# Shuijing725/CrowdNav_Prediction_AttnGraph

Hardware: AMD Instinct MI355X
Metric: env-steps/sec (sim+policy fwd) at 20 humans (higher is better)
Workload: dtype f32 (big GEMMs as bf16x3 split-precision MFMA, fp32 accumulate); 1 GPU; BASELINE configs[1]: CrowdSimVarNum-v0, 20 humans, 4096 parallel envs per GPU, HH+HR attention on, policy forward + ORCA sim step + auto-reset per step; envs_per_gpu=4096, humans=20, parallelism=dp1 (envs sharded, no rollout collective), policy_init=orthogonal, torch.manual_seed(425), sampled_actions=True, side_stream_tail=inline, dephase_steps=240

## Files before the change

crowdnav_prediction_attngraph_amd/csrc/hh_fused.hip:

```cpp
#include "hh_fused.h"
#include "row_plan.h"

#include <climits>
#include <type_traits>
#include <utility>

namespace {

typedef __bf16 bf16x8 __attribute__((ext_vector_type(8)));
typedef __bf16 bf16x4 __attribute__((ext_vector_type(4)));
typedef float f32x4 __attribute__((ext_vector_type(4)));

__device__ __forceinline__ bf16x8 ldw(const char *p)
{
    return *reinterpret_cast<const bf16x8 *>(p);
}
__device__ __forceinline__ f32x4 mfma(bf16x8 a, bf16x8 b, f32x4 c) { return __builtin_amdgcn_mfma_f32_16x16x32_bf16(a, b, c, 0, 0, 0); }

template <class F, int... I>
__device__ __forceinline__ void static_for_impl(F &&f, std::integer_sequence<int, I...>) { (f(std::integral_constant<int, I>{}), ...); }
template <int N, class F>
__device__ __forceinline__ void static_for(F &&f) { static_for_impl(f, std::make_integer_sequence<int, N>{}); }

struct Split8 { bf16x8 hi, lo; };
__device__ __forceinline__ void split1(float x, __bf16 &hi, __bf16 &lo)
{
    hi = (__bf16)x;
    lo = (__bf16)(x - (float)hi);
}
__device__ __forceinline__ Split8 split8(f32x4 a, f32x4 b)
{
    Split8 s;
#pragma unroll
    for (int q = 0; q < 4; ++q) {
        __bf16 h, l;
        split1(a[q], h, l); s.hi[q] = h; s.lo[q] = l;
        split1(b[q], h, l); s.hi[4 + q] = h; s.lo[4 + q] = l;
    }
    return s;
}

__device__ __forceinline__ int ld_ro(const int *p) { return __hip_atomic_load(p, __ATOMIC_RELAXED, __HIP_MEMORY_SCOPE_WORKGROUP); }

__device__ __forceinline__ int lower_bound_wave(const int *a, int n, int target, int lane)
{
    int lo = 0, hi = n;
    while (hi > lo) {
        const int span = hi - lo, step = (span + 63) >> 6;
        const int idx = lo + lane * step;
        const int v = idx < hi ? ld_ro(a + idx) : INT_MAX;
        const unsigned long long m = __ballot(v >= target);
        const int f = m ? __ffsll(m) - 1 : 64;
        if (f == 0) { hi = lo; }
        else {
            const int nlo = lo + (f - 1) * step + 1;
            int nhi = lo + f * step;
            nhi = nhi < hi ? nhi : hi;
            lo = nlo < nhi ? nlo : nhi; hi = nhi;
        }
    }
    return __builtin_amdgcn_readfirstlane(lo);
}

__device__ __forceinline__ int chunk_boundary(const int *row_off, int E, int total, int c, int n, int lane)
{
    if (c <= 0) return 0;
    if (c >= n) return E;
    const int target = (int)((long long)c * total / n);
    const int e1 = lower_bound_wave(row_off, E, target, lane);
    if (e1 == 0) return 0;
    const int above = ld_ro(row_off + e1) - target, below = target - ld_ro(row_off + e1 - 1);
    return below < above ? e1 - 1 : e1;
}

#ifdef HH_TIMING
__device__ long long *g_hh_tim = nullptr;
#define HH_T(k) do { const long long now_ = clock64(); tacc[k] += now_ - tlast; tlast = now_; } while (0)
#else
#define HH_T(k) do {} while (0)
#endif

struct TileCtx {
    int e_lo, n_env, r0, nrows;
    int my_env, my_start;
    int my_src, my_out;
    int tile_ord;
};

namespace wide {
constexpr int FR = 64;
constexpr int LDS_X = 0;
constexpr int LDS_S = 131072;
constexpr int LDS_H0 = LDS_S, LDS_H1 = LDS_S + 16384;
constexpr int LDS_BYTES = 163840;

template <int NRB>
__device__ __forceinline__ void tile_body(const TileCtx &t, int H, int D, const float *__restrict__ se, const HhFusedWeights &W,
                                          float *__restrict__ out_sp, char *lds, int lane, int wave)
{
    const int i = lane & 15, g = lane >> 4;
    const int loff = lane * 16;
    constexpr int NKS = (NRB + 1) / 2;
#ifdef HH_TIMING
    long long tacc[16] = {0}, tlast = clock64();
#endif

    {
        const int c0 = 32 * wave + 8 * g;
        const float *xp[NRB];
        float v[NRB][8];
#pragma unroll
        for (int rb = 0; rb < NRB; ++rb) {
            int row = rb * 16 + i;
            row = row < t.nrows ? row : t.nrows - 1;
            const int env = __shfl(t.my_env, row, 64), st = __shfl(t.my_start, row, 64);
            xp[rb] = se + ((size_t)(t.e_lo + env) * H + (row - st)) * D;
#pragma unroll
            for (int u = 0; u < 8; ++u) v[rb][u] = W.emb0_b[c0 + u];
        }
        for (int d = 0; d < D; ++d) {
            float w[8];
#pragma unroll
            for (int u = 0; u < 8; ++u) w[u] = W.emb0_w[(c0 + u) * D + d];
#pragma unroll
            for (int rb = 0; rb < NRB; ++rb) {
                const float xd = xp[rb][d];
#pragma unroll
                for (int u = 0; u < 8; ++u) v[rb][u] += xd * w[u];
            }
        }
#pragma unroll
        for (int rb = 0; rb < NRB; ++rb) {
            bf16x8 hi, lo;
#pragma unroll
            for (int u = 0; u < 8; ++u) { __bf16 h, l; split1(fmaxf(v[rb][u], 0.0f), h, l); hi[u] = h; lo[u] = l; }
            *reinterpret_cast<bf16x8 *>(lds + LDS_S + ((0 * 4 + wave) * 4 + rb) * 1024 + loff) = hi;
            *reinterpret_cast<bf16x8 *>(lds + LDS_S + ((1 * 4 + wave) * 4 + rb) * 1024 + loff) = lo;
        }
    }
    HH_T(0);
    __syncthreads();
    HH_T(1);
    {
        const char *wp = (const char *)W.emb2_frag + (size_t)wave * 4 * 16 * 1024 + loff;
#pragma unroll 1
        for (int half = 0; half < 2; ++half) {
            f32x4 acc[4][NRB];
#pragma unroll
            for (int j = 0; j < 4; ++j)
#pragma unroll
                for (int rb = 0; rb < NRB; ++rb) acc[j][rb] = f32x4{0.f, 0.f, 0.f, 0.f};
            bf16x8 wq[2][8];
#pragma unroll
            for (int j = 0; j < 4; ++j) {
                wq[0][2 * j] = ldw(wp + ((0 * 8 + half * 4 + j) * 2 + 0) * 1024);
                wq[0][2 * j + 1] = ldw(wp + ((0 * 8 + half * 4 + j) * 2 + 1) * 1024);
            }
#pragma unroll
            for (int ks = 0; ks < 4; ++ks) {
                if (ks + 1 < 4) {
#pragma unroll
                    for (int j = 0; j < 4; ++j) {
                        wq[(ks + 1) & 1][2 * j] = ldw(wp + (((ks + 1) * 8 + half * 4 + j) * 2 + 0) * 1024);
                        wq[(ks + 1) & 1][2 * j + 1] = ldw(wp + (((ks + 1) * 8 + half * 4 + j) * 2 + 1) * 1024);
                    }
                }
                bf16x8 xh[NRB], xl[NRB];
#pragma unroll
// ... 281 lines not shown
    }
    __syncthreads();
    HH_T(15);
#ifdef HH_TIMING
    if (g_hh_tim && wave == 0 && lane == 0) {
        long long *d = g_hh_tim + (size_t)blockIdx.x * 20;
        for (int k = 0; k < 16; ++k) d[k] += tacc[k];
        d[16] += 1; d[17] += t.nrows; d[18] += NRB;
        long long *d2 = g_hh_tim + (size_t)256 * 20 + ((size_t)blockIdx.x * 4 + (t.tile_ord < 3 ? t.tile_ord : 3)) * 4;
        d2[0] += tacc[4]; d2[1] += NRB; d2[2] += 1;
    }
#endif
}
}

template <int NT>
__device__ __forceinline__ void row_offsets_prologue(int E, int H, const float *__restrict__ det, int *row_off, unsigned long long *live_total, char *lds)
{
    constexpr int NW = NT / 64;
    int *part = reinterpret_cast<int *>(lds);
    const int tid = threadIdx.x, ln = tid & 63, wv = tid >> 6;
    const int chunk = (E + NT - 1) / NT;
    const int lo = tid * chunk < E ? tid * chunk : E, hi = lo + chunk < E ? lo + chunk : E;
    int sum = 0;
    for (int e = lo; e < hi; ++e) { int nd = (int)det[e]; nd = nd < 1 ? 1 : (nd > H ? H : nd); sum += nd; }
    int incl = sum;
#pragma unroll
    for (int o = 1; o < 64; o <<= 1) {
        const int v = __shfl_up(incl, o, 64);
        if (ln >= o) incl += v;
    }
    if (ln == 63) part[wv] = incl;
    __syncthreads();
    int run = incl - sum;
    for (int w = 0; w < wv; ++w) run += part[w];
    for (int e = lo; e < hi; ++e) {
        row_off[e] = run;
        int nd = (int)det[e]; nd = nd < 1 ? 1 : (nd > H ? H : nd);
        run += nd;
    }
    if (tid == NT - 1) {
        row_off[E] = run;
        if (live_total && blockIdx.x == 0) *live_total += (unsigned long long)run;
    }
    (void)NW;
    __builtin_amdgcn_fence(__ATOMIC_RELEASE, "workgroup");
    __syncthreads();
    __builtin_amdgcn_fence(__ATOMIC_ACQUIRE, "workgroup");
}

template <int FR>
__device__ __forceinline__ TileCtx next_tile(const int *row_off, int e, int e_end, int chunk_end_row, int tile_ord, int lane)
{
    TileCtx t;
    t.tile_ord = tile_ord;
    t.e_lo = e;
    t.r0 = ld_ro(row_off + e);
    const int probe = e + 1 + lane;
    const int v = probe <= e_end ? ld_ro(row_off + probe) : INT_MAX;
    const int left = chunk_end_row - t.r0;
    const int ntile = (left + FR - 1) / FR;
    const int rows = v == INT_MAX ? INT_MAX : v - t.r0;
    const bool ok = rows <= FR && left - rows <= FR * (ntile - 1);
    const int rest = left - rows;
    int key = ok ? ((((rows + 15) >> 4) + ((rest + 15) >> 4)) << 8) + (FR - rows) : INT_MAX;
    int best = key;
#pragma unroll
    for (int o = 32; o > 0; o >>= 1) { const int x = __shfl_xor(best, o, 64); best = x < best ? x : best; }
    int n_env;
    if (best == INT_MAX) {
        n_env = __popcll(__ballot(rows <= FR));
        n_env = n_env < 1 ? 1 : n_env;
    } else {
        n_env = __ffsll(__ballot(key == best));
    }
    t.n_env = n_env;
    t.nrows = __builtin_amdgcn_readfirstlane(__shfl(v, n_env - 1, 64)) - t.r0;
    const int prev_end = __shfl(v, lane >= 1 ? lane - 1 : 0, 64);
    const int st = lane >= n_env ? INT_MAX : (lane == 0 ? 0 : prev_end - t.r0);
    int cnt = 0;
    for (int k = 0; k < n_env; ++k) cnt += lane >= __builtin_amdgcn_readlane(st, k) ? 1 : 0;
    t.my_env = lane < t.nrows ? cnt - 1 : -1;
    t.my_start = __shfl(st, cnt - 1 >= 0 ? cnt - 1 : 0, 64);
    t.my_src = 0; t.my_out = t.r0 + lane;
    return t;
}

struct PlanPre { int it, out0; };
__device__ __forceinline__ PlanPre plan_prefetch(const int32_t *plan, int E, int tile, int lane)
{
    PlanPre p;
    p.it = (plan + rp_off_items(E))[(size_t)tile * 64 + lane];
    p.out0 = (plan + rp_off_rowoff())[p.it & 0xffff];
    return p;
}
__device__ __forceinline__ TileCtx plan_tile(const PlanPre &pre, int H, int tile_ord, int lane)
{
    TileCtx t;
    const unsigned long long zero = __ballot((pre.it >> 16) == 0);
    const int cnt = zero ? __ffsll((long long)zero) - 1 : 64;
    const int it = lane < cnt ? pre.it : 0;
    const int rows = it >> 16, id = it & 0xffff;
    const int out0 = pre.out0;
    int incl = rows;
#pragma unroll
    for (int o = 1; o < 64; o <<= 1) { const int y = __shfl_up(incl, o, 64); if (lane >= o) incl += y; }
    const int st = lane < cnt ? incl - rows : INT_MAX;
    t.tile_ord = tile_ord; t.e_lo = 0; t.r0 = 0; t.n_env = cnt;
    t.nrows = __builtin_amdgcn_readfirstlane(__shfl(incl, 63, 64));
    int c = 0;
    for (int k = 0; k < cnt; ++k) c += lane >= __builtin_amdgcn_readlane(st, k) ? 1 : 0;
    const int me = c - 1 >= 0 ? c - 1 : 0;
    t.my_env = lane < t.nrows ? c - 1 : -1;
    t.my_start = __shfl(st, me, 64);
    const int off = lane - t.my_start;
    t.my_src = __shfl(id, me, 64) * H + off;
    t.my_out = __shfl(out0, me, 64) + off;
    return t;
}

__global__ __launch_bounds__(256, 1) void hh_fused_wide_kernel(int E, int H, int D, const float *__restrict__ se, const float *__restrict__ det,
                                                               int *row_off, unsigned long long *live_total, HhFusedWeights W, float *__restrict__ out_sp,
                                                               unsigned long long *stamp)
{
    const CnStampScope stamp_scope(stamp);
    extern __shared__ __attribute__((aligned(16))) char lds[];
    if (det) row_offsets_prologue<256>(E, H, det, row_off, live_total, lds);
    if (stamp && blockIdx.x == 0 && threadIdx.x == 0) stamp[1] = (unsigned long long)row_off[E];
    if (W.prio) __builtin_amdgcn_s_setprio(3);
    const int lane = threadIdx.x & 63, wave = __builtin_amdgcn_readfirstlane(threadIdx.x >> 6);
    const int total = ld_ro(row_off + E);
    int e = chunk_boundary(row_off, E, total, (int)blockIdx.x, (int)gridDim.x, lane);
    const int e_end = chunk_boundary(row_off, E, total, (int)blockIdx.x + 1, (int)gridDim.x, lane);
    if (e >= e_end) return;
    int tile_ord = 0;
    const int chunk_end_row = ld_ro(row_off + e_end);
    while (e < e_end) {
        const TileCtx t = next_tile<wide::FR>(row_off, e, e_end, chunk_end_row, tile_ord++, lane);
        const int nrb = (t.nrows + 15) >> 4;
        switch (nrb) {
        case 1: wide::tile_body<1>(t, H, D, se, W, out_sp, lds, lane, wave); break;
        case 2: wide::tile_body<2>(t, H, D, se, W, out_sp, lds, lane, wave); break;
        case 3: wide::tile_body<3>(t, H, D, se, W, out_sp, lds, lane, wave); break;
        default: wide::tile_body<4>(t, H, D, se, W, out_sp, lds, lane, wave); break;
        }
        e += t.n_env;
    }
}

namespace team {

constexpr int FR = 63;
constexpr int LDS_BYTES = 163840;
template <int RB_>
struct Layout {
    static constexpr int RB = RB_;
    static constexpr bool TURNS = RB_ == 4;
    static constexpr int X_PLANE = 16 * RB * 1024;
    static constexpr int LDS_X = 0;
    static constexpr int LDS_S = 2 * X_PLANE;
    static constexpr int H_PLANE = 2 * RB * 1024;
    static constexpr int H_BYTES = 2 * H_PLANE;
    static constexpr int TEAM_S = TURNS ? 0 : 2 * H_BYTES;
    static constexpr int E0_PLANE = 4 * RB * 1024;
    static constexpr int XCH_TEAM = 4 * 2 * RB * 1024;
    static constexpr int CTR = TURNS ? LDS_X + X_PLANE + (15 * RB + 3) * 1024 + 63 * 16 : LDS_S + 4 * H_BYTES;
    static_assert(LDS_S + (TURNS ? 2 : 4) * H_BYTES + (TURNS ? 0 : 16) <= LDS_BYTES, "layout exceeds the LDS");
};

typedef __attribute__((address_space(3))) unsigned lds_u32;

typedef int i32x4 __attribute__((ext_vector_type(4)));
struct WeightBuf {
    __amdgpu_buffer_rsrc_t rs;
    unsigned emb2, qkv, os;
};
__device__ __forceinline__ WeightBuf make_weight_buf(const HhFusedWeights &W)
{
    const char *a = (const char *)W.emb2_frag, *b = (const char *)W.qkv_frag, *c = (const char *)W.os_frag;
    const char *lo = a < b ? a : b; lo = lo < c ? lo : c;
    WeightBuf wb;
    wb.rs = __builtin_amdgcn_make_buffer_rsrc((void *)lo, 0, 0x7fffffff, 0x00020000);
    wb.emb2 = (unsigned)(a - lo); wb.qkv = (unsigned)(b - lo); wb.os = (unsigned)(c - lo);
    return wb;
}
__device__ __forceinline__ bf16x8 ldb(const WeightBuf &wb, unsigned soff, unsigned voff)
{
    return __builtin_bit_cast(bf16x8, __builtin_amdgcn_raw_buffer_load_b128(wb.rs, voff, soff, 0));
}

struct RowBuf { __amdgpu_buffer_rsrc_t rs; };
__device__ __forceinline__ RowBuf make_row_buf(float *base, int r0, int nrows, int width)
{
    RowBuf rb;
    rb.rs = __builtin_amdgcn_make_buffer_rsrc((void *)(base + (size_t)r0 * width), 0, nrows * width * 4, 0x00020000);
    return rb;
}
constexpr int TRAIN_STORE_AUX = 2;
__device__ __forceinline__ void st4(const RowBuf &b, int float_off, f32x4 v)
{
    __builtin_amdgcn_raw_buffer_store_b128(__builtin_bit_cast(i32x4, v), b.rs, float_off * 4, 0, TRAIN_STORE_AUX);
}
__device__ __forceinline__ void st1(const RowBuf &b, int float_off, float v)
{
    __builtin_amdgcn_raw_buffer_store_b32(__builtin_bit_cast(int, v), b.rs, float_off * 4, 0, TRAIN_STORE_AUX);
}

__device__ __forceinline__ void team_barrier(char *lds, int bar_off, unsigned &target, int lane)
{
    lds_u32 *ctr = (lds_u32 *)(lds + bar_off);
    target += 4;
    asm volatile("s_waitcnt lgkmcnt(0)" ::: "memory");
    if (lane == 0) __hip_atomic_fetch_add(ctr, 1u, __ATOMIC_RELAXED, __HIP_MEMORY_SCOPE_WORKGROUP);
    while ((int)(__builtin_amdgcn_readfirstlane(__hip_atomic_load(ctr, __ATOMIC_RELAXED, __HIP_MEMORY_SCOPE_WORKGROUP)) - target) < 0)
        __builtin_amdgcn_s_sleep(1);
    asm volatile("" ::: "memory");
}

__device__ __forceinline__ void wait_turn(char *lds, int ctr_off, unsigned turn)
{
    lds_u32 *done = (lds_u32 *)(lds + ctr_off + 8);
    const unsigned need = 4u * turn;
    while ((int)(__builtin_amdgcn_readfirstlane(__hip_atomic_load(done, __ATOMIC_RELAXED, __HIP_MEMORY_SCOPE_WORKGROUP)) - need) < 0)
        __builtin_amdgcn_s_sleep(1);
    asm volatile("" ::: "memory");
}
__device__ __forceinline__ void finish_turn(char *lds, int ctr_off, int lane)
{
    lds_u32 *done = (lds_u32 *)(lds + ctr_off + 8);
    asm volatile("s_waitcnt lgkmcnt(0)" ::: "memory");
    if (lane == 0) __hip_atomic_fetch_add(done, 1u, __ATOMIC_RELAXED, __HIP_MEMORY_SCOPE_WORKGROUP);
}

template <int NRB, int J0, int RB>
__device__ __forceinline__ void finish_rows(const TileCtx &t, const f32x4 (&acc)[4][NRB], const char *xch, const HhFusedWeights &W,
                                            float *__restrict__ out_sp, int lane, int wave, const f32x4 *bpre = nullptr)
{
    const int i = lane & 15, g = lane >> 4, loff = lane * 16;
#pragma unroll
    for (int jj = 0; jj < 2; ++jj) {
        const int f0 = (4 * wave + J0 + jj) * 16 + 4 * g;
        const f32x4 b = bpre ? bpre[jj] : *reinterpret_cast<const f32x4 *>(W.os_b + f0);
#pragma unroll
        for (int rb = 0; rb < NRB; ++rb) {
            const f32x4 other = *reinterpret_cast<const f32x4 *>(xch + ((wave * 2 + jj) * RB + rb) * 1024 + loff);
            const int row = rb * 16 + i;
            const int orow = __shfl(t.my_out, row, 64);
            if (row < t.nrows) {
                f32x4 v = acc[J0 + jj][rb] + other + b;
#pragma unroll
                for (int q = 0; q < 4; ++q) v[q] = fmaxf(v[q], 0.0f);
                __builtin_nontemporal_store(v, reinterpret_cast<f32x4 *>(out_sp + (size_t)orow * 256 + f0));
            }
        }
    }
}

constexpr int PF = 2;

template <int NRB, bool TRAIN>
__device__ __forceinline__ void tile_body(const TileCtx &t, int H, int D, const float *__restrict__ se, const HhFusedWeights &W, const WeightBuf &WB,
                                          float *__restrict__ out_sp, char *lds, int lane_in, int wave, int tm)
{
    using L = Layout<(NRB <= 3 ? 3 : 4)>;
    constexpr int RB = L::RB, X_PLANE = L::X_PLANE, LDS_X = L::LDS_X, LDS_S = L::LDS_S, H_PLANE = L::H_PLANE, H_BYTES = L::H_BYTES,
                  E0_PLANE = L::E0_PLANE, XCH_TEAM = L::XCH_TEAM, LDS_CTR = L::CTR;
    int lane = lane_in;
    asm volatile("" : "+v"(lane));
    const int i = lane & 15, g = lane >> 4;
    const int loff = lane * 16;
    const unsigned uoff = (unsigned)loff;
    RowBuf o_e0{}, o_x{}, o_qkv{}, o_attn{};
    if (TRAIN) {
        o_e0 = make_row_buf(W.e0_out, t.r0, t.nrows, 128); o_x = make_row_buf(W.x_out, t.r0, t.nrows, 512);
        o_qkv = make_row_buf(W.qkv_out, t.r0, t.nrows, 1536); o_attn = make_row_buf(W.attn_out, t.r0, t.nrows, 512);
    }
    constexpr int NKS = (NRB + 1) / 2;
    const int w8 = 4 * tm + wave;
    RowBuf BB;
    BB.rs = __builtin_amdgcn_make_buffer_rsrc((void *)W.qkv_b, 0, 1536 * 4, 0x00020000);
#ifdef HH_TIMING
    long long tacc[16] = {0}, tlast = clock64();
#endif

    if (w8 == 0 && lane < 4) *reinterpret_cast<unsigned *>(lds + LDS_CTR + 4 * lane) = 0u;
    unsigned bar_target = 0;
    bf16x8 wq[4][8];
    {
        const int wv = w8 >> 1, half = w8 & 1;
        const unsigned wp = WB.emb2 + (unsigned)wv * 4 * 16 * 1024;
#pragma unroll
        for (int ks = 0; ks < 4; ++ks)
#pragma unroll
            for (int j = 0; j < 4; ++j) {
                wq[ks][2 * j] = ldb(WB, wp + ((ks * 8 + half * 4 + j) * 2 + 0) * 1024, uoff);
                wq[ks][2 * j + 1] = ldb(WB, wp + ((ks * 8 + half * 4 + j) * 2 + 1) * 1024, uoff);
            }
    }
    {
        const int c0 = 32 * wave + 8 * g;
#pragma unroll
        for (int rr = 0; rr < (NRB + 1) / 2; ++rr) {
            const int rb = 2 * rr + tm;
            if (rb < NRB) {
                int row = rb * 16 + i;
                row = row < t.nrows ? row : t.nrows - 1;
                const float *xp = se + (size_t)__shfl(t.my_src, row, 64) * D;
                float v[8];
#pragma unroll
                for (int u = 0; u < 8; ++u) v[u] = W.emb0_b[c0 + u];
                for (int d = 0; d < D; ++d) {
                    const float xd = xp[d];
#pragma unroll
                    for (int u = 0; u < 8; ++u) v[u] += xd * W.emb0_w[(c0 + u) * D + d];
                }
                bf16x8 hi, lo;
#pragma unroll
                for (int u = 0; u < 8; ++u) { v[u] = fmaxf(v[u], 0.0f); __bf16 h, l; split1(v[u], h, l); hi[u] = h; lo[u] = l; }
                if (TRAIN) {
                    st4(o_e0, (rb * 16 + i) * 128 + c0, f32x4{v[0], v[1], v[2], v[3]});
                    st4(o_e0, (rb * 16 + i) * 128 + c0 + 4, f32x4{v[4], v[5], v[6], v[7]});
                }
                *reinterpret_cast<bf16x8 *>(lds + LDS_S + (wave * RB + rb) * 1024 + loff) = hi;
                *reinterpret_cast<bf16x8 *>(lds + LDS_S + E0_PLANE + (wave * RB + rb) * 1024 + loff) = lo;
            }
        }
    }
    __syncthreads();
    HH_T(0);
    {
        f32x4 acc[4][NRB];
#pragma unroll
        for (int j = 0; j < 4; ++j)
#pragma unroll
            for (int rb = 0; rb < NRB; ++rb) acc[j][rb] = f32x4{0.f, 0.f, 0.f, 0.f};
#pragma unroll
        for (int ks = 0; ks < 4; ++ks) {
            bf16x8 xh[NRB], xl[NRB];
#pragma unroll
            for (int rb = 0; rb < NRB; ++rb) {
                xh[rb] = *reinterpret_cast<const bf16x8 *>(lds + LDS_S + (ks * RB + rb) * 1024 + loff);
                xl[rb] = *reinterpret_cast<const bf16x8 *>(lds + LDS_S + E0_PLANE + (ks * RB + rb) * 1024 + loff);
            }
            __builtin_amdgcn_sched_barrier(0);
            const bf16x8 *w = wq[ks];
#pragma unroll
            for (int j = 0; j < 4; ++j)
#pragma unroll
                for (int rb = 0; rb < NRB; ++rb) acc[j][rb] = mfma(w[2 * j + 1], xh[rb], acc[j][rb]);
#pragma unroll
            for (int j = 0; j < 4; ++j)
#pragma unroll
                for (int rb = 0; rb < NRB; ++rb) acc[j][rb] = mfma(w[2 * j], xl[rb], acc[j][rb]);
#pragma unroll
            for (int j = 0; j < 4; ++j)
#pragma unroll
                for (int rb = 0; rb < NRB; ++rb) acc[j][rb] = mfma(w[2 * j], xh[rb], acc[j][rb]);
            __builtin_amdgcn_sched_barrier(0);
        }
#pragma unroll
        for (int p = 0; p < 2; ++p) {
            const int fb0 = 4 * w8 + 2 * p;
            const f32x4 ba = *reinterpret_cast<const f32x4 *>(W.emb2_b + fb0 * 16 + 4 * g);
            const f32x4 bb = *reinterpret_cast<const f32x4 *>(W.emb2_b + (fb0 + 1) * 16 + 4 * g);
            const int kx = 2 * w8 + p;
#pragma unroll
            for (int rb = 0; rb < NRB; ++rb) {
                f32x4 a = acc[2 * p][rb] + ba, b = acc[2 * p + 1][rb] + bb;
#pragma unroll
                for (int q = 0; q < 4; ++q) { a[q] = fmaxf(a[q], 0.0f); b[q] = fmaxf(b[q], 0.0f); }
                if (TRAIN) {
                    st4(o_x, (rb * 16 + i) * 512 + fb0 * 16 + 4 * g, a);
                    st4(o_x, (rb * 16 + i) * 512 + fb0 * 16 + 4 * g + 16, b);
                }
                const Split8 s = split8(a, b);
                *reinterpret_cast<bf16x8 *>(lds + LDS_X + (kx * RB + rb) * 1024 + loff) = s.hi;
                if (!(L::TURNS && rb == 3 && kx == 15 && lane == 63))
                    *reinterpret_cast<bf16x8 *>(lds + LDS_X + X_PLANE + (kx * RB + rb) * 1024 + loff) = s.lo;
            }
        }
    }
    __syncthreads();
    HH_T(1);

    unsigned vmask = 0;
    {
        const int q = 16 * wave + i;
        const int eq = __shfl(t.my_env, q, 64);
#pragma unroll
        for (int jb = 0; jb < NRB; ++jb)
#pragma unroll
            for (int r = 0; r < 4; ++r) {
                const int ek = __shfl(t.my_env, 16 * jb + 4 * g + r, 64);
                if (ek == eq && eq >= 0) vmask |= 1u << (jb * 4 + r);
            }
    }

    f32x4 acc_os[4][NRB];
#pragma unroll
    for (int j = 0; j < 4; ++j)
#pragma unroll
        for (int rb = 0; rb < NRB; ++rb) acc_os[j][rb] = f32x4{0.f, 0.f, 0.f, 0.f};

    char *const H0 = lds + LDS_S + tm * L::TEAM_S, *const H1 = H0 + H_BYTES;
    const int bar = LDS_CTR + 4 * tm;
    const int h0 = ((int)blockIdx.x >> 3) & 7;
    bf16x8 wf[PF][6];
    auto ring_prologue = [&](const int hh_) __attribute__((always_inline)) {
        const unsigned wp_ = WB.qkv + (unsigned)((((h0 + 2 * hh_ + tm) & 7) * 4 + wave) * 16) * 6 * 1024;
#pragma unroll
        for (int p = 0; p < PF - 1; ++p)
#pragma unroll
            for (int c = 0; c < 6; ++c) wf[p][c] = ldb(WB, wp_ + (p * 6 + c) * 1024, uoff);
    };
    ring_prologue(0);
#pragma unroll 1
    for (int hh = 0; hh < 4; ++hh) {
        const int h = (h0 + 2 * hh + tm) & 7;
        f32x4 aq[NRB], ak[NRB], av[NRB];
#pragma unroll
        for (int rb = 0; rb < NRB; ++rb) { aq[rb] = f32x4{0.f, 0.f, 0.f, 0.f}; ak[rb] = aq[rb]; av[rb] = aq[rb]; }
        const unsigned wp = WB.qkv + (unsigned)((h * 4 + wave) * 16) * 6 * 1024;
        f32x4 bq_pf, bk_pf; float bv_pf;
        bf16x8 xh[2][NRB], xl[2][NRB];
#pragma unroll
        for (int rb = 0; rb < NRB; ++rb) {
            xh[0][rb] = *reinterpret_cast<const bf16x8 *>(lds + LDS_X + rb * 1024 + loff);
            xl[0][rb] = *reinterpret_cast<const bf16x8 *>(lds + LDS_X + X_PLANE + rb * 1024 + loff);
        }
        static_assert(16 % PF == 0, "the ring position must be compile-time inside the unrolled group");
        auto group = [&](const int k4, auto tail_c) __attribute__((always_inline)) {
        constexpr bool TAIL = decltype(tail_c)::value;
        static_for<PF>([&](auto ku_c) __attribute__((always_inline)) {
            constexpr int ku = decltype(ku_c)::value;
            const int ks = k4 + ku;
            {
                if (!TAIL || ku == 0) {
#pragma unroll
                    for (int c = 0; c < 6; ++c) wf[(ku + PF - 1) % PF][c] = ldb(WB, wp + ((ks + PF - 1) * 6 + c) * 1024, uoff);
                }
                if (!TAIL || ku + 1 < PF) {
#pragma unroll
// ... 150 lines not shown
        if (wave < NRB) {
#pragma unroll
            for (int ks = 0; ks < NKS; ++ks) {
                const Split8 sp = split8(f32x4{p[2 * ks][0], p[2 * ks][1], p[2 * ks][2], p[2 * ks][3]},
                                         f32x4{p[2 * ks + 1][0], p[2 * ks + 1][1], p[2 * ks + 1][2], p[2 * ks + 1][3]});
                *reinterpret_cast<bf16x8 *>(H0 + (ks * RB + wave) * 1024 + loff) = sp.hi;
                *reinterpret_cast<bf16x8 *>(H0 + H_PLANE + (ks * RB + wave) * 1024 + loff) = sp.lo;
            }
        }
        team_barrier(lds, bar, bar_target, lane);
        HH_T(7);
        f32x4 o[NRB];
#pragma unroll
        for (int ib = 0; ib < NRB; ++ib) o[ib] = f32x4{0.f, 0.f, 0.f, 0.f};
#pragma unroll
        for (int ks = 0; ks < NKS; ++ks) {
            const Split8 vf = split8(av[2 * ks], 2 * ks + 1 < NRB ? av[2 * ks + 1 < NRB ? 2 * ks + 1 : 0] : f32x4{0.f, 0.f, 0.f, 0.f});
#pragma unroll
            for (int ib = 0; ib < NRB; ++ib) {
                const bf16x8 ph = *reinterpret_cast<const bf16x8 *>(H0 + (ks * RB + ib) * 1024 + loff);
                const bf16x8 pl = *reinterpret_cast<const bf16x8 *>(H0 + H_PLANE + (ks * RB + ib) * 1024 + loff);
                o[ib] = mfma(vf.lo, ph, o[ib]);
                o[ib] = mfma(vf.hi, pl, o[ib]);
                o[ib] = mfma(vf.hi, ph, o[ib]);
            }
        }
#pragma unroll
        for (int ib = 0; ib < NRB; ++ib) {
            if (TRAIN) st4(o_attn, (ib * 16 + i) * 512 + h * 64 + 16 * wave + 4 * g, o[ib]);
            bf16x4 oh, ol;
#pragma unroll
            for (int q = 0; q < 4; ++q) { __bf16 a, b; split1(o[ib][q], a, b); oh[q] = a; ol[q] = b; }
            const int off = ((wave >> 1) * RB + ib) * 1024 + loff + 8 * (wave & 1);
            *reinterpret_cast<bf16x4 *>(H1 + off) = oh;
            *reinterpret_cast<bf16x4 *>(H1 + H_PLANE + off) = ol;
        }
        HH_T(8);
        team_barrier(lds, bar, bar_target, lane);
        HH_T(9);
#pragma unroll
        for (int ks = 0; ks < 2; ++ks) {
            bf16x8 oh[NRB], ol[NRB];
#pragma unroll
            for (int rb = 0; rb < NRB; ++rb) {
                oh[rb] = *reinterpret_cast<const bf16x8 *>(H1 + (ks * RB + rb) * 1024 + loff);
                ol[rb] = *reinterpret_cast<const bf16x8 *>(H1 + H_PLANE + (ks * RB + rb) * 1024 + loff);
            }
#pragma unroll
            for (int j = 0; j < 4; ++j)
#pragma unroll
                for (int rb = 0; rb < NRB; ++rb) acc_os[j][rb] = mfma(wos[ks][j][1], oh[rb], acc_os[j][rb]);
#pragma unroll
            for (int j = 0; j < 4; ++j)
#pragma unroll
                for (int rb = 0; rb < NRB; ++rb) acc_os[j][rb] = mfma(wos[ks][j][0], ol[rb], acc_os[j][rb]);
#pragma unroll
            for (int j = 0; j < 4; ++j)
#pragma unroll
                for (int rb = 0; rb < NRB; ++rb) acc_os[j][rb] = mfma(wos[ks][j][0], oh[rb], acc_os[j][rb]);
            if (L::TURNS && ks == 1) finish_turn(lds, LDS_CTR, lane);
        }
        __builtin_amdgcn_s_setprio(1);
        HH_T(10);
    }
    f32x4 bfin[2];
#pragma unroll
    for (int jj = 0; jj < 2; ++jj) bfin[jj] = *reinterpret_cast<const f32x4 *>(W.os_b + (4 * wave + 2 * tm + jj) * 16 + 4 * g);
    __syncthreads();
    HH_T(11);
    {
        char *const xch = lds + LDS_X;
        if (tm == 0) {
#pragma unroll
            for (int jj = 0; jj < 2; ++jj)
#pragma unroll
                for (int rb = 0; rb < NRB; ++rb) *reinterpret_cast<f32x4 *>(xch + ((wave * 2 + jj) * RB + rb) * 1024 + loff) = acc_os[2 + jj][rb];
        } else {
#pragma unroll
            for (int jj = 0; jj < 2; ++jj)
#pragma unroll
                for (int rb = 0; rb < NRB; ++rb) *reinterpret_cast<f32x4 *>(xch + XCH_TEAM + ((wave * 2 + jj) * RB + rb) * 1024 + loff) = acc_os[jj][rb];
        }
        __syncthreads();
        if (tm == 0) finish_rows<NRB, 0, RB>(t, acc_os, xch + XCH_TEAM, W, out_sp, lane, wave, bfin);
        else finish_rows<NRB, 2, RB>(t, acc_os, xch, W, out_sp, lane, wave, bfin);
    }
    HH_T(12);
#ifdef HH_TIMING
    if (g_hh_tim && wave == 0 && lane == 0) {
        long long *d = g_hh_tim + ((size_t)blockIdx.x * 2 + tm) * 20;
        for (int k = 0; k < 16; ++k) d[k] += tacc[k];
        d[16] += 1; d[17] += t.nrows; d[18] += NRB;
    }
#endif
}

}

template <bool TRAIN>
__global__ __launch_bounds__(512, 2) void hh_fused_kernel(int E, int H, int D, const float *__restrict__ se, const float *__restrict__ det,
                                                          int *row_off, unsigned long long *live_total, HhFusedWeights W, float *__restrict__ out_sp,
                                                          const int32_t *__restrict__ plan, unsigned long long *stamp)
{
    const CnStampScope stamp_scope(TRAIN ? nullptr : stamp);
    extern __shared__ __attribute__((aligned(16))) char lds[];
#ifdef HH_TIMING
    const long long k_c0 = clock64(), k_r0 = wall_clock64();
#endif
    bool planned = !TRAIN && det && rp_usable(plan, E, H) && plan[1] == (int)gridDim.x;
    if (planned) {
        const int32_t *pro = plan + rp_off_rowoff();
        int bad = 0;
        for (int i = (int)threadIdx.x; i < E; i += (int)blockDim.x) {
            int nd = (int)det[i]; nd = nd < 1 ? 1 : (nd > H ? H : nd);
            bad |= (pro[i + 1] - pro[i]) ^ nd;
        }
        volatile int *flag = reinterpret_cast<volatile int *>(lds);
        if (threadIdx.x == 0) *flag = 0;
        __syncthreads();
        if (__ballot(bad != 0) != 0ull && (threadIdx.x & 63) == 0) *flag = 1;
        __syncthreads();
        planned = __builtin_amdgcn_readfirstlane(*flag) == 0;
        __syncthreads();
    }
    if (det && !planned) row_offsets_prologue<512>(E, H, det, row_off, live_total, lds);
    if (!TRAIN && stamp && blockIdx.x == 0 && threadIdx.x == 0) stamp[1] = (unsigned long long)(planned ? plan[3] : row_off[E]);
#ifdef HH_TIMING
    const long long k_c1 = clock64();
#endif
    __builtin_amdgcn_s_setprio(1);
    const int lane = threadIdx.x & 63, w8 = __builtin_amdgcn_readfirstlane(threadIdx.x >> 6);
    const int wave = w8 & 3, tm = w8 >> 2;
    int e = 0, e_end = 0, chunk_end_row = 0, n_plan = 0;
    PlanPre pre{0, 0};
    if (planned) {
        if (live_total && blockIdx.x == 0 && threadIdx.x == 0) *live_total += (unsigned long long)plan[3];
        n_plan = plan[2];
        pre = plan_prefetch(plan, E, (int)blockIdx.x, lane);
        for (int i = (int)(blockIdx.x * blockDim.x + threadIdx.x); i <= E; i += (int)(gridDim.x * blockDim.x)) row_off[i] = plan[rp_off_rowoff() + i];
    } else {
        const int total = ld_ro(row_off + E);
        e = chunk_boundary(row_off, E, total, (int)blockIdx.x, (int)gridDim.x, lane);
        e_end = chunk_boundary(row_off, E, total, (int)blockIdx.x + 1, (int)gridDim.x, lane);
        if (e >= e_end) return;
        chunk_end_row = ld_ro(row_off + e_end);
    }
    int tile_ord = 0;
    const team::WeightBuf WB = team::make_weight_buf(W);
    for (;;) {
        TileCtx t;
        if (planned) {
            if (tile_ord >= n_plan) break;
            const PlanPre cur = pre;
            ++tile_ord;
            if (tile_ord < n_plan) pre = plan_prefetch(plan, E, (int)blockIdx.x + tile_ord * (int)gridDim.x, lane);
            t = plan_tile(cur, H, tile_ord - 1, lane);
            if (t.nrows == 0) continue;
        } else {
            if (e >= e_end) break;
            t = next_tile<team::FR>(row_off, e, e_end, chunk_end_row, tile_ord++, lane);
            t.my_src = (t.e_lo + t.my_env) * H + (lane - t.my_start);
            e += t.n_env;
        }
        const int nrb = (t.nrows + 15) >> 4;
        switch (nrb) {
        case 1: team::tile_body<1, TRAIN>(t, H, D, se, W, WB, out_sp, lds, lane, wave, tm); break;
        case 2: team::tile_body<2, TRAIN>(t, H, D, se, W, WB, out_sp, lds, lane, wave, tm); break;
        case 3: team::tile_body<3, TRAIN>(t, H, D, se, W, WB, out_sp, lds, lane, wave, tm); break;
        default: team::tile_body<4, TRAIN>(t, H, D, se, W, WB, out_sp, lds, lane, wave, tm); break;
        }
    }
#ifdef HH_TIMING
    if (g_hh_tim && (threadIdx.x & 255) == 0) {
        long long *d = g_hh_tim + ((size_t)blockIdx.x * 2 + (threadIdx.x >> 8)) * 20;
        d[13] += clock64() - k_c0; d[14] += wall_clock64() - k_r0; d[15] += k_c1 - k_c0;
    }
#endif
}

__device__ __forceinline__ int koff(int g, int u, bool perm) { return perm ? 16 * (u >> 2) + 4 * g + (u & 3) : 8 * g + u; }

__device__ __forceinline__ void bake_emb2(int idx, const float *__restrict__ w, __bf16 *__restrict__ out)
{
    if (idx >= 512 * 128) return;
    const int u = idx & 7, lane = (idx >> 3) & 63, j = (idx >> 9) & 7, ks = (idx >> 12) & 3, wv = idx >> 14;
    const int fb = 8 * wv + j;
    const float x = w[(size_t)(fb * 16 + (lane & 15)) * 128 + 32 * ks + koff(lane >> 4, u, false)];
    const __bf16 hi = (__bf16)x;
    const size_t base = ((((size_t)wv * 4 + ks) * 8 + j) * 2) * 512 + lane * 8 + u;
    out[base] = hi;
    out[base + 512] = (__bf16)(x - (float)hi);
}
__device__ __forceinline__ void bake_qkv(int idx, const float *__restrict__ w, __bf16 *__restrict__ out)
{
    if (idx >= 1536 * 512) return;
    const int u = idx & 7, lane = (idx >> 3) & 63;
    int rest = idx >> 9;
    const int j = rest % 3; rest /= 3;
    const int ks = rest & 15, wv = (rest >> 4) & 3, h = rest >> 6;
    const int sec = j == 2 ? 2 : (wv & 1), blk = j == 2 ? wv : (wv & ~1) + j;
    const float x = w[(size_t)(sec * 512 + h * 64 + 16 * blk + (lane & 15)) * 512 + 32 * ks + koff(lane >> 4, u, true)];
    const __bf16 hi = (__bf16)x;
    const size_t base = (((((size_t)h * 4 + wv) * 16 + ks) * 3 + j) * 2) * 512 + lane * 8 + u;
    out[base] = hi;
    out[base + 512] = (__bf16)(x - (float)hi);
}
__device__ __forceinline__ void bake_os(int idx, const float *__restrict__ w, __bf16 *__restrict__ out)
{
    if (idx >= 256 * 512) return;
    const int u = idx & 7, lane = (idx >> 3) & 63, j = (idx >> 9) & 3, ks = (idx >> 11) & 1, wv = (idx >> 12) & 3, h = idx >> 14;
    const float x = w[(size_t)((4 * wv + j) * 16 + (lane & 15)) * 512 + h * 64 + 32 * ks + koff(lane >> 4, u, true)];
    const __bf16 hi = (__bf16)x;
    const size_t base = (((((size_t)h * 4 + wv) * 2 + ks) * 4 + j) * 2) * 512 + lane * 8 + u;
    out[base] = hi;
    out[base + 512] = (__bf16)(x - (float)hi);
}

__global__ void bake_all_kernel(const float *__restrict__ emb2_w, const float *__restrict__ qkv_w, const float *__restrict__ os_w, __bf16 *__restrict__ emb2_frag,
                                __bf16 *__restrict__ qkv_frag, __bf16 *__restrict__ os_frag)
{
    constexpr int B1 = 512 * 128 / 256, B2 = B1 + 1536 * 512 / 256;
    const int b = blockIdx.x;
    if (b < B1) bake_emb2(b * 256 + (int)threadIdx.x, emb2_w, emb2_frag);
    else if (b < B2) bake_qkv((b - B1) * 256 + (int)threadIdx.x, qkv_w, qkv_frag);
    else bake_os((b - B2) * 256 + (int)threadIdx.x, os_w, os_frag);
}

}

int hh_fused_bake(const float *emb2_w, const float *qkv_w, const float *os_w, void *emb2_frag, void *qkv_frag, void *os_frag, hipStream_t st)
{
    hipLaunchKernelGGL(bake_all_kernel, dim3((512 * 128 + 1536 * 512 + 256 * 512) / 256), dim3(256), 0, st, emb2_w, qkv_w, os_w, (__bf16 *)emb2_frag, (__bf16 *)qkv_frag,
                       (__bf16 *)os_frag);
    CN_CHECK_LAUNCH();
    return CN_OK;
}

#ifdef HH_TIMING
extern "C" int cn_hh_fused_set_timing(long long *buf)
{
    CN_HIP(hipMemcpyToSymbol(HIP_SYMBOL(g_hh_tim), &buf, sizeof(buf)));
    return CN_OK;
}
#endif

int hh_fused_forward(int E, int H, int D, const float *spatial_edges, const float *det, int *row_off, unsigned long long *live_total,
                     const HhFusedWeights &w, float *out_sp, hipStream_t st, const int32_t *row_plan)
{
    unsigned long long *stamp = cn_stamp_slot(CN_K_HH_FUSED);
    static thread_local int attr_dev = -1;
    int dev = 0;
    CN_HIP(hipGetDevice(&dev));
    if (dev != attr_dev) {
// ... 20 lines not shown
```

Baseline: 15.56 million env-steps/s.

## Overlap plan and emb0 loads with weight fetch in team HH kernel

Moves the next tile's plan-item load and the output-row-offset lookup into the tile body, issuing them early so their latency hides behind the emb2 weight loads and first MFMAs. The per-row emb0 input/weight loads are hoisted and batched across row blocks with software pipelining before the weight-register loads. The kernel prologue's plan validation now loads det and row offsets into registers in a fixed unrolled batch and uses a per-wave flag array instead of a strided loop with three barriers. The cost is higher register pressure and more complex scheduling with sched_barrier and held() pins.

```diff
diff --git a/crowdnav_prediction_attngraph_amd/csrc/hh_fused.hip b/crowdnav_prediction_attngraph_amd/csrc/hh_fused.hip
--- a/crowdnav_prediction_attngraph_amd/csrc/hh_fused.hip
+++ b/crowdnav_prediction_attngraph_amd/csrc/hh_fused.hip
@@ -83,7 +83,8 @@
 struct TileCtx {
     int e_lo, n_env, r0, nrows;
     int my_env, my_start;
-    int my_src, my_out;
+    int my_src;
+    int out0, it;
     int tile_ord;
 };
 
@@ -531,26 +532,19 @@
     for (int k = 0; k < n_env; ++k) cnt += lane >= __builtin_amdgcn_readlane(st, k) ? 1 : 0;
     t.my_env = lane < t.nrows ? cnt - 1 : -1;
     t.my_start = __shfl(st, cnt - 1 >= 0 ? cnt - 1 : 0, 64);
-    t.my_src = 0; t.my_out = t.r0 + lane;
+    t.my_src = 0;
+    t.out0 = t.r0 + (lane < n_env ? st : 0); t.it = 0;
     return t;
 }
 
-struct PlanPre { int it, out0; };
-__device__ __forceinline__ PlanPre plan_prefetch(const int32_t *plan, int E, int tile, int lane)
-{
-    PlanPre p;
-    p.it = (plan + rp_off_items(E))[(size_t)tile * 64 + lane];
-    p.out0 = (plan + rp_off_rowoff())[p.it & 0xffff];
-    return p;
-}
-__device__ __forceinline__ TileCtx plan_tile(const PlanPre &pre, int H, int tile_ord, int lane)
+constexpr int PLAN_NONE = -2, PLAN_LAST = -1;
+__device__ __forceinline__ TileCtx plan_tile(int item, int H, int tile_ord, int lane)
 {
     TileCtx t;
-    const unsigned long long zero = __ballot((pre.it >> 16) == 0);
+    const unsigned long long zero = __ballot((item >> 16) == 0);
     const int cnt = zero ? __ffsll((long long)zero) - 1 : 64;
-    const int it = lane < cnt ? pre.it : 0;
+    const int it = lane < cnt ? item : 0;
     const int rows = it >> 16, id = it & 0xffff;
-    const int out0 = pre.out0;
     int incl = rows;
 #pragma unroll
     for (int o = 1; o < 64; o <<= 1) { const int y = __shfl_up(incl, o, 64); if (lane >= o) incl += y; }
@@ -564,7 +558,7 @@
     t.my_start = __shfl(st, me, 64);
     const int off = lane - t.my_start;
     t.my_src = __shfl(id, me, 64) * H + off;
-    t.my_out = __shfl(out0, me, 64) + off;
+    t.out0 = 0; t.it = item;
     return t;
 }
 
@@ -682,7 +676,7 @@
 }
 
 template <int NRB, int J0, int RB>
-__device__ __forceinline__ void finish_rows(const TileCtx &t, const f32x4 (&acc)[4][NRB], const char *xch, const HhFusedWeights &W,
+__device__ __forceinline__ void finish_rows(const TileCtx &t, int my_out, const f32x4 (&acc)[4][NRB], const char *xch, const HhFusedWeights &W,
                                             float *__restrict__ out_sp, int lane, int wave, const f32x4 *bpre = nullptr)
 {
     const int i = lane & 15, g = lane >> 4, loff = lane * 16;
@@ -694,7 +688,7 @@
         for (int rb = 0; rb < NRB; ++rb) {
             const f32x4 other = *reinterpret_cast<const f32x4 *>(xch + ((wave * 2 + jj) * RB + rb) * 1024 + loff);
             const int row = rb * 16 + i;
-            const int orow = __shfl(t.my_out, row, 64);
+            const int orow = __shfl(my_out, row, 64);
             if (row < t.nrows) {
                 f32x4 v = acc[J0 + jj][rb] + other + b;
 #pragma unroll
@@ -709,7 +703,7 @@
 
 template <int NRB, bool TRAIN>
 __device__ __forceinline__ void tile_body(const TileCtx &t, int H, int D, const float *__restrict__ se, const HhFusedWeights &W, const WeightBuf &WB,
-                                          float *__restrict__ out_sp, char *lds, int lane_in, int wave, int tm)
+                                          float *__restrict__ out_sp, char *lds, int lane_in, int wave, int tm, const int32_t *__restrict__ plan, int plan_next, int &it_next)
 {
     using L = Layout<(NRB <= 3 ? 3 : 4)>;
     constexpr int RB = L::RB, X_PLANE = L::X_PLANE, LDS_X = L::LDS_X, LDS_S = L::LDS_S, H_PLANE = L::H_PLANE, H_BYTES = L::H_BYTES,
@@ -734,10 +728,56 @@
 
     if (w8 == 0 && lane < 4) *reinterpret_cast<unsigned *>(lds + LDS_CTR + 4 * lane) = 0u;
     unsigned bar_target = 0;
+    constexpr int NRR = (NRB + 1) / 2;
+    const int c0 = 32 * wave + 8 * g;
+    const float *xp[NRR];
+    float v[NRR][8];
+    float xv[NRR][4], wv[8][4], bv0[8];
+    auto e0_load = [&](const int d0, const int q0, const int q1) __attribute__((always_inline)) {
+#pragma unroll
+        for (int q = q0; q < q1; ++q) {
+#pragma unroll
+            for (int rr = 0; rr < NRR; ++rr) xv[rr][q] = xp[rr][d0 + q];
+#pragma unroll
+            for (int u = 0; u < 8; ++u) wv[u][q] = W.emb0_w[(c0 + u) * D + d0 + q];
+        }
+    };
+    auto e0_fma = [&](const int q0, const int q1) __attribute__((always_inline)) {
+#pragma unroll
+        for (int q = q0; q < q1; ++q)
+#pragma unroll
+            for (int rr = 0; rr < NRR; ++rr)
+#pragma unroll
+                for (int u = 0; u < 8; ++u) v[rr][u] += xv[rr][q] * wv[u][q];
+    };
+#pragma unroll
+    for (int rr = 0; rr < NRR; ++rr) {
+        int row = (2 * rr + tm) * 16 + i;
+        row = row < t.nrows ? row : t.nrows - 1;
+        xp[rr] = se + (size_t)__shfl(t.my_src, row, 64) * D;
+    }
+#pragma unroll
+    for (int q = 0; q < 4; ++q) {
+#pragma unroll
+        for (int rr = 0; rr < NRR; ++rr) xv[rr][q] = 0.0f;
+#pragma unroll
+        for (int u = 0; u < 8; ++u) wv[u][q] = 0.0f;
+    }
+    {
+        const int q1 = D >= 2 ? 1 : 0;
+#pragma unroll
+        for (int rr = 0; rr < NRR; ++rr) { xv[rr][0] = xp[rr][0]; xv[rr][1] = xp[rr][q1]; }
+#pragma unroll
+        for (int u = 0; u < 8; ++u) { wv[u][0] = W.emb0_w[(c0 + u) * D]; wv[u][1] = W.emb0_w[(c0 + u) * D + q1]; }
+    }
+    if (D >= 4) e0_load(0, 2, 4);
+#pragma unroll
+    for (int u = 0; u < 8; ++u) bv0[u] = W.emb0_b[c0 + u];
+    __builtin_amdgcn_sched_barrier(0);
     bf16x8 wq[4][8];
     {
-        const int wv = w8 >> 1, half = w8 & 1;
-        const unsigned wp = WB.emb2 + (unsigned)wv * 4 * 16 * 1024;
+        const int wv_ = w8 >> 1, half = w8 & 1;
+        const unsigned wp = WB.emb2 + (unsigned)wv_ * 4 * 16 * 1024;
 #pragma unroll
         for (int ks = 0; ks < 4; ++ks)
 #pragma unroll
@@ -746,29 +786,47 @@
                 wq[ks][2 * j + 1] = ldb(WB, wp + ((ks * 8 + half * 4 + j) * 2 + 1) * 1024, uoff);
             }
     }
+    int out0_ld, it_ld;
+    const int pnext = TRAIN ? PLAN_NONE : __builtin_amdgcn_readfirstlane(plan_next);
+    const bool has_plan = pnext != PLAN_NONE, has_next = pnext >= 0;
     {
-        const int c0 = 32 * wave + 8 * g;
-#pragma unroll
-        for (int rr = 0; rr < (NRB + 1) / 2; ++rr) {
+        const int32_t *dummy = reinterpret_cast<const int32_t *>(se);
+        out0_ld = *(has_plan ? plan + rp_off_rowoff() + (t.it & 0xffff) : dummy);
+        it_ld = *(has_next ? plan + pnext + lane : dummy);
+    }
+    __builtin_amdgcn_sched_barrier(0);
+#pragma unroll
+    for (int rr = 0; rr < NRR; ++rr)
+#pragma unroll
+        for (int q = 0; q < 4; ++q) xv[rr][q] = held(xv[rr][q]);
+#pragma unroll
+    for (int u = 0; u < 8; ++u) {
+        bv0[u] = held(bv0[u]);
+#pragma unroll
+        for (int q = 0; q < 4; ++q) wv[u][q] = held(wv[u][q]);
+    }
+    {
+#pragma unroll
+        for (int rr = 0; rr < NRR; ++rr)
+#pragma unroll
+            for (int u = 0; u < 8; ++u) v[rr][u] = bv0[u];
+        e0_fma(0, 1);
+        if (D >= 2) e0_fma(1, 2);
+        if (D >= 4) e0_fma(2, 4);
+        int d0 = 4;
+        for (; d0 + 4 <= D; d0 += 4) { e0_load(d0, 0, 4); e0_fma(0, 4); }
+        if (d0 + 2 <= D) { e0_load(d0, 0, 2); e0_fma(0, 2); }
+        if ((D & 1) && D > 1) { e0_load(D - 1, 0, 1); e0_fma(0, 1); }
+#pragma unroll
+        for (int rr = 0; rr < NRR; ++rr) {
             const int rb = 2 * rr + tm;
             if (rb < NRB) {
-                int row = rb * 16 + i;
-                row = row < t.nrows ? row : t.nrows - 1;
-                const float *xp = se + (size_t)__shfl(t.my_src, row, 64) * D;
-                float v[8];
-#pragma unroll
-                for (int u = 0; u < 8; ++u) v[u] = W.emb0_b[c0 + u];
-                for (int d = 0; d < D; ++d) {
-                    const float xd = xp[d];
-#pragma unroll
-                    for (int u = 0; u < 8; ++u) v[u] += xd * W.emb0_w[(c0 + u) * D + d];
-                }
                 bf16x8 hi, lo;
 #pragma unroll
-                for (int u = 0; u < 8; ++u) { v[u] = fmaxf(v[u], 0.0f); __bf16 h, l; split1(v[u], h, l); hi[u] = h; lo[u] = l; }
+                for (int u = 0; u < 8; ++u) { v[rr][u] = fmaxf(v[rr][u], 0.0f); __bf16 h, l; split1(v[rr][u], h, l); hi[u] = h; lo[u] = l; }
                 if (TRAIN) {
-                    st4(o_e0, (rb * 16 + i) * 128 + c0, f32x4{v[0], v[1], v[2], v[3]});
-                    st4(o_e0, (rb * 16 + i) * 128 + c0 + 4, f32x4{v[4], v[5], v[6], v[7]});
+                    st4(o_e0, (rb * 16 + i) * 128 + c0, f32x4{v[rr][0], v[rr][1], v[rr][2], v[rr][3]});
+                    st4(o_e0, (rb * 16 + i) * 128 + c0 + 4, f32x4{v[rr][4], v[rr][5], v[rr][6], v[rr][7]});
                 }
                 *reinterpret_cast<bf16x8 *>(lds + LDS_S + (wave * RB + rb) * 1024 + loff) = hi;
                 *reinterpret_cast<bf16x8 *>(lds + LDS_S + E0_PLANE + (wave * RB + rb) * 1024 + loff) = lo;
@@ -777,6 +835,7 @@
     }
     __syncthreads();
     HH_T(0);
+    int my_out;
     {
         f32x4 acc[4][NRB];
 #pragma unroll
@@ -807,6 +866,9 @@
                 for (int rb = 0; rb < NRB; ++rb) acc[j][rb] = mfma(w[2 * j], xh[rb], acc[j][rb]);
             __builtin_amdgcn_sched_barrier(0);
         }
+        out0_ld = held(out0_ld); it_ld = held(it_ld);
+        it_next = has_next ? it_ld : 0;
+        my_out = __shfl(has_plan ? out0_ld : t.out0, t.my_env >= 0 ? t.my_env : 0, 64) + (lane - t.my_start);
 #pragma unroll
         for (int p = 0; p < 2; ++p) {
             const int fb0 = 4 * w8 + 2 * p;
@@ -1123,8 +1185,8 @@
                 for (int rb = 0; rb < NRB; ++rb) *reinterpret_cast<f32x4 *>(xch + XCH_TEAM + ((wave * 2 + jj) * RB + rb) * 1024 + loff) = acc_os[jj][rb];
         }
         __syncthreads();
-        if (tm == 0) finish_rows<NRB, 0, RB>(t, acc_os, xch + XCH_TEAM, W, out_sp, lane, wave, bfin);
-        else finish_rows<NRB, 2, RB>(t, acc_os, xch, W, out_sp, lane, wave, bfin);
+        if (tm == 0) finish_rows<NRB, 0, RB>(t, my_out, acc_os, xch + XCH_TEAM, W, out_sp, lane, wave, bfin);
+        else finish_rows<NRB, 2, RB>(t, my_out, acc_os, xch, W, out_sp, lane, wave, bfin);
     }
     HH_T(12);
 #ifdef HH_TIMING
@@ -1148,68 +1210,102 @@
 #ifdef HH_TIMING
     const long long k_c0 = clock64(), k_r0 = wall_clock64();
 #endif
-    bool planned = !TRAIN && det && rp_usable(plan, E, H) && plan[1] == (int)gridDim.x;
-    if (planned) {
+    const int tid = (int)threadIdx.x, lane = tid & 63, w8 = __builtin_amdgcn_readfirstlane(tid >> 6);
+    const int wave = w8 & 3, tm = w8 >> 2;
+    bool planned = false;
+    int n_plan = 0;
+    int it_cur = 0;
+    if (!TRAIN && det && plan && E >= 1 && E <= RP_EMAX && H <= RP_HMAX) {
+        struct alignas(16) Hdr { int32_t w[RP_HDR]; };
         const int32_t *pro = plan + rp_off_rowoff();
-        int bad = 0;
-        for (int i = (int)threadIdx.x; i < E; i += (int)blockDim.x) {
-            int nd = (int)det[i]; nd = nd < 1 ? 1 : (nd > H ? H : nd);
-            bad |= (pro[i + 1] - pro[i]) ^ nd;
-        }
-        volatile int *flag = reinterpret_cast<volatile int *>(lds);
-        if (threadIdx.x == 0) *flag = 0;
-        __syncthreads();
-        if (__ballot(bad != 0) != 0ull && (threadIdx.x & 63) == 0) *flag = 1;
-        __syncthreads();
-        planned = __builtin_amdgcn_readfirstlane(*flag) == 0;
-        __syncthreads();
+        const Hdr hdr = *reinterpret_cast<const Hdr *>(plan);
+        it_cur = (plan + rp_off_items(E))[(size_t)blockIdx.x * 64 + lane];
+        constexpr int VU = RP_EMAX / 512;
+        float dv[VU];
+        int pa[VU], pb[VU];
+#pragma unroll
+        for (int k = 0; k < VU; ++k) {
+            const int i = tid + 512 * k, ic = i < E ? i : E - 1;
+            dv[k] = det[ic]; pa[k] = pro[ic]; pb[k] = pro[ic + 1];
+        }
+        const int ci = (int)blockIdx.x * 512 + tid;
+        int cpy = pro[ci <= E ? ci : 0];
+#pragma unroll
+        for (int k = 0; k < VU; ++k) { dv[k] = held(dv[k]); pa[k] = held(pa[k]); pb[k] = held(pb[k]); }
+        cpy = held(cpy); it_cur = held(it_cur);
+        const bool shaped = hdr.w[0] == RP_MAGIC && hdr.w[4] == E && hdr.w[5] == H && hdr.w[1] == (int)gridDim.x;
+        if (shaped) {
+            int bad = 0;
+#pragma unroll
+            for (int k = 0; k < VU; ++k) {
+                int nd = (int)dv[k]; nd = nd < 1 ? 1 : (nd > H ? H : nd);
+                bad |= (pb[k] - pa[k]) ^ nd;
+            }
+            team::lds_u32 *vw = (team::lds_u32 *)lds;
+            const unsigned wbad = __ballot(bad != 0) != 0ull ? 1u : 0u;
+            if (lane == 0) vw[w8] = wbad;
+            __syncthreads();
+            unsigned any = 0;
+#pragma unroll
+            for (int k = 0; k < 8; ++k) any |= vw[k];
+            planned = __builtin_amdgcn_readfirstlane(any) == 0;
+            if (!planned) __syncthreads();
+        }
+        if (planned) {
+            n_plan = hdr.w[2];
+            if (ci <= E) row_off[ci] = cpy;
+            for (int i = ci + (int)gridDim.x * 512; i <= E; i += (int)gridDim.x * 512) row_off[i] = pro[i];
+            if (blockIdx.x == 0 && tid == 0) {
+                if (stamp) stamp[1] = (unsigned long long)hdr.w[3];
+                if (live_total) atomicAdd(live_total, (unsigned long long)hdr.w[3]);
+            }
+        }
     }
     if (det && !planned) row_offsets_prologue<512>(E, H, det, row_off, live_total, lds);
-    if (!TRAIN && stamp && blockIdx.x == 0 && threadIdx.x == 0) stamp[1] = (unsigned long long)(planned ? plan[3] : row_off[E]);
+    if (!TRAIN && !planned && stamp && blockIdx.x == 0 && tid == 0) stamp[1] = (unsigned long long)row_off[E];
 #ifdef HH_TIMING
     const long long k_c1 = clock64();
 #endif
     __builtin_amdgcn_s_setprio(1);
-    const int lane = threadIdx.x & 63, w8 = __builtin_amdgcn_readfirstlane(threadIdx.x >> 6);
-    const int wave = w8 & 3, tm = w8 >> 2;
-    int e = 0, e_end = 0, chunk_end_row = 0, n_plan = 0;
-    PlanPre pre{0, 0};
-    if (planned) {
-        if (live_total && blockIdx.x == 0 && threadIdx.x == 0) *live_total += (unsigned long long)plan[3];
-        n_plan = plan[2];
-        pre = plan_prefetch(plan, E, (int)blockIdx.x, lane);
-        for (int i = (int)(blockIdx.x * blockDim.x + threadIdx.x); i <= E; i += (int)(gridDim.x * blockDim.x)) row_off[i] = plan[rp_off_rowoff() + i];
-    } else {
+    int e = 0, e_end = 0, chunk_end_row = 0;
+    if (!planned) {
         const int total = ld_ro(row_off + E);
         e = chunk_boundary(row_off, E, total, (int)blockIdx.x, (int)gridDim.x, lane);
         e_end = chunk_boundary(row_off, E, total, (int)blockIdx.x + 1, (int)gridDim.x, lane);
         if (e >= e_end) return;
-        chunk_end_row = ld_ro(row_off + e_end);
+        chunk_end_row = __builtin_amdgcn_readfirstlane(ld_ro(row_off + e_end));
     }
     int tile_ord = 0;
     const team::WeightBuf WB = team::make_weight_buf(W);
     for (;;) {
         TileCtx t;
+        int it_next = 0;
+        int plan_next = PLAN_NONE;
+        int ln = lane;
+        asm volatile("" : "+v"(ln));
         if (planned) {
             if (tile_ord >= n_plan) break;
-            const PlanPre cur = pre;
             ++tile_ord;
-            if (tile_ord < n_plan) pre = plan_prefetch(plan, E, (int)blockIdx.x + tile_ord * (int)gridDim.x, lane);
-            t = plan_tile(cur, H, tile_ord - 1, lane);
-            if (t.nrows == 0) continue;
+            plan_next = tile_ord < n_plan ? rp_off_items(E) + ((int)blockIdx.x + tile_ord * (int)gridDim.x) * 64 : PLAN_LAST;
+            t = plan_tile(it_cur, H, tile_ord - 1, ln);
+            if (t.nrows == 0) {
+                it_cur = plan_next >= 0 ? plan[plan_next + ln] : 0;
+                continue;
+            }
         } else {
             if (e >= e_end) break;
-            t = next_tile<team::FR>(row_off, e, e_end, chunk_end_row, tile_ord++, lane);
-            t.my_src = (t.e_lo + t.my_env) * H + (lane - t.my_start);
+            t = next_tile<team::FR>(row_off, e, e_end, chunk_end_row, tile_ord++, ln);
+            t.my_src = (t.e_lo + t.my_env) * H + (ln - t.my_start);
             e += t.n_env;
         }
         const int nrb = (t.nrows + 15) >> 4;
         switch (nrb) {
-        case 1: team::tile_body<1, TRAIN>(t, H, D, se, W, WB, out_sp, lds, lane, wave, tm); break;
-        case 2: team::tile_body<2, TRAIN>(t, H, D, se, W, WB, out_sp, lds, lane, wave, tm); break;
-        case 3: team::tile_body<3, TRAIN>(t, H, D, se, W, WB, out_sp, lds, lane, wave, tm); break;
-        default: team::tile_body<4, TRAIN>(t, H, D, se, W, WB, out_sp, lds, lane, wave, tm); break;
-        }
+        case 1: team::tile_body<1, TRAIN>(t, H, D, se, W, WB, out_sp, lds, lane, wave, tm, plan, plan_next, it_next); break;
+        case 2: team::tile_body<2, TRAIN>(t, H, D, se, W, WB, out_sp, lds, lane, wave, tm, plan, plan_next, it_next); break;
+        case 3: team::tile_body<3, TRAIN>(t, H, D, se, W, WB, out_sp, lds, lane, wave, tm, plan, plan_next, it_next); break;
+        default: team::tile_body<4, TRAIN>(t, H, D, se, W, WB, out_sp, lds, lane, wave, tm, plan, plan_next, it_next); break;
+        }
+        it_cur = it_next;
     }
 #ifdef HH_TIMING
     if (g_hh_tim && (threadIdx.x & 255) == 0) {
```

Result: faster. 15.74 million env-steps/s, median of 6 (+1.2%).
